# AshuiRUA/NPI-GNN

Hardware: AMD Instinct MI355X
Metric: edges/sec per GNN layer (fwd+bwd) (higher is better)
Workload: dtype f32; 1 GPU; C4 synthetic ncRNA-protein bipartite graph, N=1000000 nodes, E=20000000 directed edges (both directions, Zipf-skewed protein side), 1 SAGEConv layer 256->256 fp32, fwd+bwd incl. dX/dW/db, graph+features resident in HBM; parallelism=single GPU, hip_graph_replay=False, setup_steps=40, csr_sorted_columns=True

## Files before the change

include/npi_gnn.h:

```cpp
#ifndef NPI_GNN_H
#define NPI_GNN_H

#include <stdint.h>

#ifdef __cplusplus
extern "C" {
#endif

#define NPI_OK 0
#define NPI_ERR_ARG (-1)
#define NPI_ERR_LAUNCH (-2)
#define NPI_ERR_WORKSPACE (-3)

#ifndef NPI_ITEM_EDGES
#define NPI_ITEM_EDGES 256
#endif

#define NPI_F32 0
#define NPI_BF16 1

const char* npi_last_error(void);
int npi_abi_version(void);

int64_t npi_csr_workspace_bytes(int64_t E, int64_t N);
// ... 5 lines not shown
int npi_csr_build_ex(const int64_t* key_nodes, const int64_t* val_nodes, int64_t E, int64_t N,
                     int64_t n_cols, int add_self_loops, int64_t loop_col_offset, int build_flags,
                     int32_t* rowptr, int32_t* col, int32_t* eid, int32_t* rowidx,
                     int32_t* item_row, int64_t item_edges, int32_t* status,
                     void* workspace, int64_t workspace_bytes, void* stream);

int npi_edge_positions(const int32_t* eid, const int32_t* rowptr, int64_t N, int64_t nnz_max,
                       int64_t E, int32_t* pos_of, void* stream);

int64_t npi_segsum_carry_elems(int64_t nnz_max, int64_t item_edges, int64_t F);
int npi_segsum_scales_supported(int64_t F, int dtype);
int npi_segsum_ex(const int32_t* rowptr, const int32_t* col, const int32_t* item_row, int64_t item_edges,
                   const float* w, int64_t N, int64_t nnz_max, const void* x, int64_t ldx,
                   const void* x2, int64_t split, void* out, int64_t ldo, int64_t F, int dtype, int mean,
                   const float* bias, float* carry, float* row_scales_out, void* stream);

int npi_row_weight_sum(const int32_t* rowptr, const float* w, int64_t N, float* deg, void* stream);
int npi_gcn_norm(const int32_t* rowidx, const int32_t* col, const int32_t* rowptr, const float* w,
                 const float* deg, const int32_t* deg_rowptr, int64_t N, int64_t nnz_max, float* norm,
                 void* stream);
int npi_entry_col_scale(const int32_t* col, const int32_t* rowptr, const float* table, const float* w_in, int64_t N, int64_t n_cols,
                        int64_t nnz_max, float* w_out, void* stream);
int npi_row_inv_count(const int32_t* rowptr, int64_t N, float* inv_cnt, void* stream);
int npi_entry_weights(const int32_t* eid, const int32_t* rowidx, const int32_t* rowptr,
                      const float* edge_w, const float* loop_w_node, float fill,
                      int64_t N, int64_t nnz_max, float* w_entry, void* stream);
int npi_hold_cus(int workgroups, int64_t nanoseconds, uint64_t* start_word, void* stream);
int npi_relu_backward(const float* dy, int64_t ldd, const float* y, int64_t ldy, int64_t M, int64_t F, float* dz, int64_t ldz,
                      void* stream);

// ... 189 lines not shown
```

npi_gnn_amd/_lib.py:

```python
from __future__ import annotations

import ctypes
import os
from ctypes import c_char_p, c_float, c_int, c_int64, c_void_p

import torch

HERE = os.path.dirname(os.path.abspath(__file__))
LIB_PATH = os.environ.get("NPI_GNN_LIB") or os.path.join(HERE, "libnpi_gnn.so")

NPI_F32 = 0
NPI_BF16 = 1
NPI_GEMM_EXACT_F32 = 1
NPI_GEMM_SPLIT_BF16 = 2
NPI_GEMM_A_ZERO_PADDED = 4
NPI_GEMM_WORKSPACE_PREPARED = 8
NPI_GEMM_SPLIT_F16X2 = 16
NPI_PREPARE_F16X2 = 4


def NPI_GEMM_RESERVE_CUS(n: int) -> int:
    n = int(n)
    if n < 0 or n > 128 or n % 8:
        raise ValueError(f"NPI_GEMM_RESERVE_CUS: a multiple of 8 in [0, 128], got {n}")
    return (n // 8) << 8

_P = c_void_p
_I = c_int64

PROTOTYPES = {
    "npi_last_error": (c_char_p, []),
    "npi_abi_version": (c_int, []),
    "npi_csr_workspace_bytes": (_I, [_I, _I]),
    "npi_item_edges": (_I, [_I]),
    "npi_num_items": (_I, [_I, _I]),
    "npi_csr_build_ex": (c_int, [_P, _P, _I, _I, _I, c_int, _I, c_int, _P, _P, _P, _P, _P, _I, _P, _P, _I, _P]),
    "npi_edge_positions": (c_int, [_P, _P, _I, _I, _I, _P, _P]),
    "npi_segsum_carry_elems": (_I, [_I, _I, _I]),
    "npi_segsum_ex": (c_int, [_P, _P, _P, _I, _P, _I, _I, _P, _I, _P, _I, _P, _I, _I, c_int, c_int, _P, _P, _P, _P]),
    "npi_segsum_scales_supported": (c_int, [_I, c_int]),
    "npi_row_weight_sum": (c_int, [_P, _P, _I, _P, _P]),
    "npi_gcn_norm": (c_int, [_P, _P, _P, _P, _P, _P, _I, _I, _P, _P]),
    "npi_row_inv_count": (c_int, [_P, _I, _P, _P]),
    "npi_entry_col_scale": (c_int, [_P, _P, _P, _P, _I, _I, _I, _P, _P]),
    "npi_entry_weights": (c_int, [_P, _P, _P, _P, _P, c_float, _I, _I, _P, _P]),
    "npi_relu_backward": (c_int, [_P, _I, _P, _I, _I, _I, _P, _I, _P]),
    "npi_l2_normalize_rows": (c_int, [_P, _I, _I, _I, c_float, _P, _I, _P, _P]),
    "npi_l2_normalize_rows_bwd": (c_int, [_P, _I, _P, _I, _P, _I, _I, c_float, _P, _I, _P]),
    "npi_colsum_workspace_elems": (_I, [_I, _I]),
    "npi_colsum": (c_int, [_P, _I, _I, _I, _P, _P, _I, _P]),
    "npi_linear_bwd_weight_workspace_elems": (_I, [_I, _I, _I]),
    "npi_linear_workspace_bytes": (_I, [_I, _I]),
    "npi_row_scales": (c_int, [_P, _I, _I, _I, _P, _P]),
    "npi_linear_fwd_ex": (c_int, [_P, _I, _P, _I, _P, _P, _P, _I, _I, _I, _I, c_int, c_int, c_int, _P, _I, _P, _P]),
    "npi_linear_bwd_data_ex": (c_int, [_P, _I, _P, _I, _P, _P, _I, _I, _I, _I, c_int, c_int, _P, _I, _P, _P]),
# ... 124 lines not shown
```

npi_gnn_amd/build.py:

```python
from __future__ import annotations

import os
import shutil
import subprocess
import sys

HERE = os.path.dirname(os.path.abspath(__file__))
CSRC = os.path.join(HERE, "csrc")
LIB = os.path.join(HERE, "libnpi_gnn.so")
SOURCES = ["csr_build.hip", "segsum.hip", "gemm_f32.hip", "graph_ops.hip", "gat.hip", "segscan.hip", "pool.hip", "subgraph.hip",
           "head.hip", "layer.hip"]
HOST_ONLY = {"layer.hip"}
ARCH = "gfx950"


def _hipcc() -> str:
    for cand in (os.environ.get("HIPCC"), shutil.which("hipcc"), "/opt/rocm/bin/hipcc"):
        if cand and os.path.exists(cand):
            return cand
    raise RuntimeError("hipcc not found (expected /opt/rocm/bin/hipcc)")


MANIFEST = os.path.join(HERE, "build", "manifest.json")


# ... 64 lines not shown
```

npi_gnn_amd/csrc/csr_build.hip:

```cpp
#include "npi_common.h"
#include <stdarg.h>

namespace npi {

static thread_local char g_err[512] = "";
void set_error(const char* fmt, ...) {
    va_list ap;
    va_start(ap, fmt);
    vsnprintf(g_err, sizeof(g_err), fmt, ap);
    va_end(ap);
}

constexpr int SORT_THREADS = 256;
constexpr int SORT_WAVES = SORT_THREADS / WAVE;
constexpr int SORT_ITEMS = 16;
constexpr int SORT_WAVE_TILE = WAVE * SORT_ITEMS;
constexpr int SORT_TILE = SORT_THREADS * SORT_ITEMS;
constexpr int RADIX = 256;

constexpr int SCAN_THREADS = 256;
constexpr int SCAN_ITEMS = 8;
constexpr int SCAN_TILE = SCAN_THREADS * SCAN_ITEMS;
static_assert(SCAN_THREADS == SORT_THREADS && SORT_THREADS == 256, "one thread per radix digit");

// ... 579 lines not shown
    if (n_out == 0) {
        (void)hipMemsetAsync(rowptr_o, 0, sizeof(int32_t), stream);
    } else {
        const unsigned tiles = (unsigned)ceil_div(n_out, 256);
        int32_t* cnt = workspace;
        int32_t* tile_total = workspace + n_out;
        csr_filter_count_kernel<<<tiles, 256, 0, stream>>>(rowptr, col, perm, remap, (int)n_out, cnt, tile_total);
        csr_filter_fill_kernel<<<tiles, 256, 0, stream>>>(rowptr, col, eid, perm, remap, newpos, (int)n_out, cnt, tile_total,
                                                          rowptr_o, col_o, eid_o, rowidx_o);
    }
    const int64_t n_items = num_items_of(nnz_max_out, item_edges);
    item_rows_kernel<<<(unsigned)ceil_div(n_items + 1, 256), 256, 0, stream>>>(rowptr_o, n_out, n_items, (int)item_edges, item_row_o);
    return check_launch("npi_csr_filter");
}

extern "C" int npi_edge_positions(const int32_t* eid, const int32_t* rowptr, int64_t N, int64_t nnz_max,
                                  int64_t E, int32_t* pos_of, void* stream_) {
    hipStream_t stream = (hipStream_t)stream_;
    NPI_REQUIRE(E >= 0 && nnz_max >= 0, "npi_edge_positions: negative size");
    if (E > 0) fill_i32_kernel<<<(unsigned)ceil_div(E, 256), 256, 0, stream>>>(pos_of, E, -1);
    if (nnz_max > 0)
        edge_positions_kernel<<<(unsigned)ceil_div(nnz_max, 256), 256, 0, stream>>>(eid, rowptr, N, nnz_max, pos_of);
    return check_launch("npi_edge_positions");
}
```

npi_gnn_amd/functional.py:

```python
from __future__ import annotations

from typing import Optional

import torch

from ._lib import (NPI_BF16, NPI_F32, NPI_GEMM_A_ZERO_PADDED, NPI_GEMM_EXACT_F32, NPI_GEMM_RESERVE_CUS, NPI_GEMM_SPLIT_F16X2,
                   NPI_GEMM_WORKSPACE_PREPARED, NPI_PREPARE_F16X2, check, load, ptr, require_gpu, stream_ptr)
from .graph import CSRGraph, CSRSide, as_graph
from .schedule import DEFAULT, Schedule


_PROFILE = None
_PROFILE_TAGS = None


class _tag_events:

    def __init__(self, tag, dev):
        self.rec = _PROFILE_TAGS
        if self.rec is not None:
            self.tag, self.dev = tag, dev
            self.e0, self.e1 = torch.cuda.Event(enable_timing=True), torch.cuda.Event(enable_timing=True)

    def __enter__(self):
# ... 73 lines not shown
def _check_out(out: torch.Tensor, rows: int, cols: int, like: torch.Tensor, what: str) -> None:
    if (out.dim() != 2 or out.size(0) != rows or out.size(1) != cols or out.dtype != like.dtype or out.stride(1) != 1
            or out.device != like.device):
        raise ValueError(f"{what}: out must be [{rows}, {cols}] {like.dtype} with unit column stride on {like.device} "
                         f"(got {tuple(out.shape)} {out.dtype}, strides {tuple(out.stride())}, {out.device})")


def segsum_scales_ok(side: CSRSide, x: torch.Tensor, out: Optional[torch.Tensor] = None) -> bool:
    return (x.dtype == torch.float32 and x.size(1) == 256 and side.nnz_max > 0 and x.stride(0) % 4 == 0 and x.data_ptr() % 16 == 0
            and (out is None or (out.stride(0) % 4 == 0 and out.data_ptr() % 16 == 0)))


def segsum(graph: CSRGraph, side: CSRSide, x: torch.Tensor, w: Optional[torch.Tensor] = None,
           mean: bool = False, bias: Optional[torch.Tensor] = None,
           out: Optional[torch.Tensor] = None, x2: Optional[torch.Tensor] = None,
           scales_out: Optional[torch.Tensor] = None) -> torch.Tensor:
    dev = require_gpu(x, w, bias, x2)
    x = _fcp(x, "x")
    if bias is not None:
        bias = _fc(bias, "bias", x)
    N, F = side.n_rows, x.size(1)
    split = x.size(0)
    if x2 is not None:
        x2 = _fc(x2, "x2", x)
        if x2.size(1) != F:
            raise ValueError("x2 must have the width of x")
        if x2.stride(0) != x.stride(0):
            x2 = x2.contiguous()
            if x2.stride(0) != x.stride(0):
                x = x.contiguous()
    if side.n_cols > split + (x2.size(0) if x2 is not None else 0):
        raise ValueError(f"the table has {split + (x2.size(0) if x2 is not None else 0)} rows, the adjacency indexes {side.n_cols}")
    if out is None:
        out = torch.empty((N, F), dtype=x.dtype, device=dev)
    else:
        _check_out(out, N, F, x, "segsum")
    carry = side.carry(F)
    prof = _PROFILE
    if prof is not None:
        ev0, ev1 = torch.cuda.Event(enable_timing=True), torch.cuda.Event(enable_timing=True)
        ev0.record(torch.cuda.current_stream(dev))
    if scales_out is not None and (scales_out.dtype != torch.float32 or scales_out.numel() != N or not scales_out.is_contiguous()):
        raise ValueError("segsum: scales_out must be a contiguous float32 vector with one element per output row")
    check(load().npi_segsum_ex(ptr(side.rowptr), ptr(side.col), ptr(side.item_row), side.item, ptr(w), N, side.nnz_max,
                                ptr(x), x.stride(0), ptr(x2), split if x2 is not None else 0, ptr(out), out.stride(0), F,
                                _code(x), 1 if mean else 0, ptr(bias), ptr(carry), ptr(scales_out), stream_ptr(dev)), "npi_segsum")
    if prof is not None:
        ev1.record(torch.cuda.current_stream(dev))
        prof.append((ev0, ev1))
    return out




def _gflags(sch: Schedule) -> int:
    return NPI_GEMM_EXACT_F32 if sch.gemm_exact_f32 else 0


def _f16x2(sch: Schedule, rows: int, K: int, N: int, dtype) -> bool:
    return (sch.f16x2_min_rows is not None and not sch.gemm_exact_f32 and rows >= sch.f16x2_min_rows and dtype == torch.float32
            and f16x2_shape(rows, K, N))


def _gemm_workspace(K: int, N: int, dev) -> torch.Tensor:
    return torch.empty(int(load().npi_linear_workspace_bytes(K, N)), dtype=torch.uint8, device=dev)
# ... 428 lines not shown
    inv = graph.inv_count(graph.by_dst)
    out = torch.empty(max(tside.nnz_max, 1), dtype=torch.float32, device=dev)
    check(load().npi_entry_col_scale(ptr(tside.col), ptr(tside.rowptr), ptr(inv), ptr(w_src), tside.n_rows, inv.numel(), tside.nnz_max,
                                     ptr(out), stream_ptr(dev)), "npi_entry_col_scale")
    if w_src is None:
        cache[key] = out
    return out


def _aggregate_first_ok(sch: Schedule, f16: bool, weight: torch.Tensor, grad_out: torch.Tensor, tside: CSRSide, ws_bwd) -> bool:
    return (sch.aggregate_first_backward and f16 and isinstance(ws_bwd, Planes) and ws_bwd.f16 and grad_out.dtype == torch.float32 and grad_out.size(1) == 256
            and segsum_scales_ok(tside, grad_out) and f16x2_shape(grad_out.size(0), grad_out.size(1), weight.size(0)))


def _backward_aggregate_first(graph, tside: CSRSide, w_t: Optional[torch.Tensor], agg, weight, grad_out, ws_bwd: "Planes", want_w: bool,
                              has_bias: bool, overlap: bool, k_valid=None):
    dev = grad_out.device
    N, Nout = grad_out.shape
    t = torch.empty((N, Nout), dtype=torch.float32, device=dev)
    t_scales = torch.empty(N, dtype=torch.float32, device=dev)
    dw = db = None
    if overlap and want_w:
        main = torch.cuda.current_stream(dev)
        side = _side_stream(dev)
        side.wait_stream(main)
        dw, db = linear_bwd_weight(agg, grad_out, want_bias=has_bias, shared=True, k_valid=k_valid)
        with torch.cuda.stream(side):
            segsum(graph, tside, grad_out, w=w_t, mean=False, out=t, scales_out=t_scales)
        for buf in (grad_out, t, t_scales):
            buf.record_stream(side)
        main.wait_stream(side)
    else:
        if want_w:
            dw, db = linear_bwd_weight(agg, grad_out, want_bias=has_bias, k_valid=k_valid)
        segsum(graph, tside, grad_out, w=w_t, mean=False, out=t, scales_out=t_scales)
    dx = linear_bwd_data(t, weight, ws=ws_bwd, dc_scales=t_scales)
    return dx, dw, db


class _SageConvFn(torch.autograd.Function):
    @staticmethod
    def forward(ctx, x, weight, bias, graph: CSRGraph, w_entry=None, relu: bool = False, sch: Schedule = DEFAULT):
        ctx.graph = graph
        ctx.w_src = w_entry[1] if w_entry else None
        ctx.has_bias = bias is not None
        ctx.relu = relu
        ctx.sch = sch
        ctx.k_rows = None
        f16 = (x.dtype == weight.dtype and x.size(1) == weight.size(0)
               and _f16x2(sch, graph.by_dst.n_rows, weight.size(0), weight.size(1), x.dtype) and segsum_scales_ok(graph.by_dst, x))
        ctx.f16 = f16
        if f16:
            agg = torch.empty((graph.by_dst.n_rows, x.size(1)), dtype=x.dtype, device=x.device)
            scales = torch.empty(agg.size(0), dtype=torch.float32, device=x.device)
            segsum(graph, graph.by_dst, x, w=w_entry[0] if w_entry else None, mean=True, out=agg, scales_out=scales)
            wsf, ctx.ws_bwd = prepare_weight(weight, backward=ctx.needs_input_grad[0], f16=True)
            out = linear_fwd(agg, weight, bias, relu=relu, ws=wsf, a_scales=scales)
            ctx.k_valid = None
            ctx.save_for_backward(agg, weight, *([out] if relu else []))
            return out
        fl = _gflags(sch)
        if not fl and _layer_calls_ok() and x.dtype == weight.dtype and x.dtype in (torch.float32, torch.bfloat16) and not (
                x.dtype == torch.bfloat16 and weight.size(0) % 128 != 0 and 2 * _pad128(weight.size(0)) <= 3 * weight.size(0)):
            agg, out, ctx.ws_bwd = conv_fwd(graph.by_dst, x, w_entry[0] if w_entry else None, True, weight, bias, relu,
                                            ctx.needs_input_grad[0])
            ctx.k_valid = weight.size(0) if agg.size(1) != weight.size(0) else None
            ctx.save_for_backward(agg, weight, *([out] if relu else []))
            return out
        agg = None if fl else padded_aggregate_buffer(x, weight.size(0), graph.by_dst.n_rows, bf16_ok=True)
        if agg is None:
            agg = segsum(graph, graph.by_dst, x, w=w_entry[0] if w_entry else None, mean=True)
        else:
            segsum(graph, graph.by_dst, x, w=w_entry[0] if w_entry else None, mean=True, out=agg[:, : x.size(1)])
        if agg.size(1) != weight.size(0) and agg.dtype == torch.bfloat16:
            ctx.k_rows = weight.size(0)
            weight = torch.nn.functional.pad(weight.detach(), (0, 0, 0, agg.size(1) - weight.size(0)))
        wsf, ctx.ws_bwd = prepare_weight(weight, backward=ctx.needs_input_grad[0]) if (
            agg.size(1) == weight.size(0) and agg.dtype == weight.dtype and not fl) else (None, None)
        out = linear_fwd(agg, weight, bias, relu=relu, ws=wsf, flags=fl)
        ctx.k_valid = weight.size(0) if agg.size(1) != weight.size(0) else None
        ctx.save_for_backward(agg, weight, *([out] if relu else []))
        return out

    @staticmethod
    def backward(ctx, grad_out):
        agg, weight = ctx.saved_tensors[:2]
# ... 7 lines not shown
        if not fl and not overlap and ctx.k_rows is None and _layer_calls_ok() and (want_w or want_x) and not ctx.f16:
            out_relu = None
            if ctx.relu:
                if grad_out.dtype == torch.float32:
                    out_relu = ctx.saved_tensors[2]
                else:
                    grad_out = relu_backward(grad_out, ctx.saved_tensors[2])
            dx, dw, db = conv_bwd(tside() if want_x else graph.by_dst, grad_out, out_relu, agg, weight, graph.inv_count(graph.by_dst),
                                  ctx.w_src, ctx.ws_bwd, want_x, want_w, ctx.has_bias)
            return dx, dw, db, None, None, None, None
        if ctx.relu:
            grad_out = relu_backward(grad_out, ctx.saved_tensors[2])
        dx = dw = db = None
        if want_x and _aggregate_first_ok(ctx.sch, ctx.f16, weight, grad_out, tside(), ctx.ws_bwd):
            ts = tside()
            dx, dw, db = _backward_aggregate_first(graph, ts, mean_bwd_weights(graph, ts, ctx.w_src), agg, weight, grad_out, ctx.ws_bwd,
                                                   want_w, ctx.has_bias, overlap, ctx.k_valid)
            return dx, dw, db, None, None, None, None
        ws_bwd = ctx.ws_bwd if not (isinstance(ctx.ws_bwd, Planes) and ctx.ws_bwd.f16) else None
        if want_w and not overlap:
            dw, db = linear_bwd_weight(agg, grad_out, want_bias=ctx.has_bias, k_valid=ctx.k_valid, flags=fl)
        if want_x:
            dagg = linear_bwd_data(grad_out, weight, rowscale=graph.inv_count(graph.by_dst), ws=ws_bwd, flags=fl)
            if ctx.k_rows is not None:
                dagg = dagg[:, : ctx.k_rows]
            if overlap:
                dev = grad_out.device
                main = torch.cuda.current_stream(dev)
                side = _side_stream(dev)
                side.wait_stream(main)
                dw, db = linear_bwd_weight(agg, grad_out, want_bias=ctx.has_bias, shared=True, k_valid=ctx.k_valid, flags=fl)
                with torch.cuda.stream(side):
                    dx = segsum(graph, tside(), dagg, w=ctx.w_src, mean=False)
                dagg.record_stream(side)
                dx.record_stream(main)
                main.wait_stream(side)
            else:
                dx = segsum(graph, tside(), dagg, w=ctx.w_src, mean=False)
        if dw is not None and ctx.k_rows is not None:
            dw = dw[: ctx.k_rows]
        return dx, dw, db, None, None, None, None


class _SageConcatFn(torch.autograd.Function):

    @staticmethod
    def forward(ctx, x, weight, bias, graph: CSRGraph, w_entry=None):
        N, F = x.shape
        cat = torch.empty((N, 2 * F), dtype=x.dtype, device=x.device)
        cat[:, :F].copy_(x)
        segsum(graph, graph.by_dst, x, w=w_entry[0] if w_entry else None, mean=True, out=cat[:, F:])
        out = linear_fwd(cat, weight, bias)
        ctx.graph, ctx.F = graph, F
# ... 724 lines not shown
```

npi_gnn_amd/graph.py:

```python
from __future__ import annotations

from dataclasses import dataclass, field
from typing import Dict, Optional

import torch

from . import _lib
from ._lib import check, load, ptr, require_gpu, stream_ptr

_DEBUG = False

_PENDING = []
_PENDING_MAX = 256


def set_debug(flag: bool) -> None:
    global _DEBUG
    _DEBUG = bool(flag)


def pending_status(device=None) -> list:
    if device is None:
        out = list(_PENDING)
        _PENDING.clear()
# ... 40 lines not shown
@dataclass
class CSRSide:
    rowptr: torch.Tensor
    col: torch.Tensor
    eid: torch.Tensor
    rowidx: torch.Tensor
    item_row: torch.Tensor
    status: torch.Tensor
    nnz_max: int
    n_items: int
    _inv_cnt: Optional[torch.Tensor] = None
    _carry: Dict[tuple, torch.Tensor] = field(default_factory=dict)
    n_rows: int = -1
    n_cols: int = -1
    item: int = 0

    def inv_count(self) -> torch.Tensor:
        if self._inv_cnt is None:
            dev = self.rowptr.device
            out = torch.empty(self.n_rows, dtype=torch.float32, device=dev)
            check(load().npi_row_inv_count(ptr(self.rowptr), self.n_rows, ptr(out), stream_ptr(dev)),
                  "npi_row_inv_count")
            self._inv_cnt = out
        return self._inv_cnt

    def carry(self, F: int) -> torch.Tensor:
        dev = self.rowptr.device
        key = (F, _lib.stream_ptr(dev))
        buf = self._carry.pop(key, None)
        if buf is None:
            n = int(load().npi_segsum_carry_elems(self.nnz_max, self.item, F))
            buf = torch.zeros(n, dtype=torch.float32, device=dev)
            if len(self._carry) >= CARRY_SLOTS and not torch.cuda.is_current_stream_capturing():
                self._carry.pop(next(iter(self._carry)))
        elif _DEBUG and not torch.cuda.is_current_stream_capturing():
            self._check_counters(buf)
        self._carry[key] = buf
        return buf

    def _check_counters(self, buf: torch.Tensor) -> None:
        n_wg = -(-self.n_items // 4)
        n = n_wg + 2 * (-(-n_wg // 64))
        if n and int(buf[:n].view(torch.int32).abs().max()) != 0:
            raise _lib.NpiError("aggregation scratch: an arrival counter is not zero between launches -- two launches shared the "
                                "buffer concurrently or one was aborted; call reset_carry() on this side")

    def reset_carry(self) -> None:
        self._carry.clear()


def item_hint(nnz_max: int) -> int:
    return int(load().npi_item_edges(int(nnz_max)))


def build_side(key: torch.Tensor, val: torch.Tensor, n_rows: int, n_cols: int, self_loops: bool = True,
               loop_col_offset: int = 0, drop_equal: bool = True, item: Optional[int] = None,
               sort_columns: bool = False) -> CSRSide:
    lib = load()
    dev = require_gpu(key, val)
    E, N = int(key.numel()), int(n_rows)
    nnz_max = E + (N if self_loops else 0)
    item = item_hint(nnz_max) if item is None else int(item)
    n_items = int(lib.npi_num_items(nnz_max, item))
# ... 9 lines not shown
    ws_bytes = int(lib.npi_csr_workspace_bytes(E, N))
    ws = torch.empty(ws_bytes, dtype=torch.uint8, device=dev)
    check(lib.npi_csr_build_ex(ptr(key), ptr(val), E, N, int(n_cols), 1 if self_loops else 0,
                               int(loop_col_offset), (1 if drop_equal else 0) | (2 if sort_columns else 0), ptr(rowptr), ptr(col), ptr(eid),
                               ptr(rowidx), ptr(item_row), item, ptr(status), ptr(ws), ws_bytes, stream_ptr(dev)),
          "npi_csr_build_ex")
    note_status(status)
    side = CSRSide(rowptr, col, eid, rowidx, item_row, status, nnz_max, n_items)
    side.n_rows, side.n_cols, side.item = N, int(n_cols), item
    return side


class CSRGraph:

    def __init__(self, edge_index: torch.Tensor, num_nodes: int, self_loops: bool = True, by_dst: Optional[CSRSide] = None,
                 symmetric: bool = False, item: Optional[int] = None, sort_columns: bool = False, keep_equal: bool = False):
        if edge_index.dtype != torch.int64 or edge_index.dim() != 2 or edge_index.size(0) != 2:
            raise ValueError("edge_index must be a LongTensor of shape [2, E]")
        require_gpu(edge_index)
        self.num_nodes = int(num_nodes)
        self.num_edges = int(edge_index.size(1))
        self.self_loops = bool(self_loops)
        self.device = edge_index.device
        self._ei_version = edge_index._version
        self._ei_ptr = edge_index.data_ptr()
        self.symmetric = bool(symmetric)
        self._src = edge_index[0].contiguous()
        self._dst = edge_index[1].contiguous()
        self._item = item if by_dst is None else by_dst.item
        self.sort_columns = bool(sort_columns)
        self.keep_equal = bool(keep_equal)
        if self.keep_equal and self.self_loops:
            raise ValueError("CSRGraph: keep_equal=True (existing self loops stay ordinary entries) needs self_loops=False")
        self.by_dst = by_dst if by_dst is not None else \
            build_side(self._dst, self._src, self.num_nodes, self.num_nodes, self.self_loops, drop_equal=not self.keep_equal,
                       item=self._item, sort_columns=self.sort_columns)
        self._by_src: Optional[CSRSide] = None

    @property
    def by_src(self) -> CSRSide:
        if self._by_src is None:
            self._by_src = build_side(self._src, self._dst, self.num_nodes, self.num_nodes, self.self_loops,
                                      drop_equal=not self.keep_equal, item=self.by_dst.item, sort_columns=self.sort_columns)
        return self._by_src

    def built_from(self, edge_index: torch.Tensor, num_nodes: Optional[int] = None) -> bool:
# ... 159 lines not shown
```

Before: 3.207 billion edges/s.

## Stream hub rows as dense masked column scan instead of CSR gather

Picks up to 128 highest-degree rows (hubs) of the CSR side and builds a per-column bitmask of which hubs touch each column. A new streaming kernel walks the feature table once in slabs and accumulates all hub rows at the same time from shared-memory tiles. The remaining light rows are aggregated by the existing segsum on a reduced CSR. This targets the cost of Zipf-skewed hub rows, which cause long serial gathers and load imbalance. In exchange it adds a full dense pass over X, partial buffers and a finalize step, plus a one-time planning cost and a host sync when the plan is built.

```diff
diff --git a/include/npi_gnn.h b/include/npi_gnn.h
--- a/include/npi_gnn.h
+++ b/include/npi_gnn.h
@@ -43,6 +43,20 @@
                    const float* w, int64_t N, int64_t nnz_max, const void* x, int64_t ldx,
                    const void* x2, int64_t split, void* out, int64_t ldo, int64_t F, int dtype, int mean,
                    const float* bias, float* carry, float* row_scales_out, void* stream);
+
+#define NPI_HUB_MAX 128
+int64_t npi_hub_plan_workspace_elems(void);
+int npi_hub_plan(const int32_t* rowptr, const int32_t* col, int64_t N, int64_t n_cols, int64_t nnz_max, int64_t h_max,
+                 int64_t min_degree, int64_t min_entries, int32_t* hub_rows, uint32_t* mask, int32_t* info, int32_t* workspace,
+                 void* stream);
+int npi_hub_light_side(const int32_t* rowptr, const int32_t* col, const int32_t* eid, const int32_t* rowidx, int64_t N,
+                       int64_t nnz_max, const int32_t* hub_rows, int64_t H, int64_t nnz_max_light, int64_t item_edges,
+                       int32_t* rowptr_l, int32_t* col_l, int32_t* eid_l, int32_t* rowidx_l, int32_t* item_row_l, void* stream);
+int64_t npi_segsum_hub_slabs(int64_t n_cols);
+int64_t npi_segsum_hub_partial_elems(int64_t n_cols);
+int npi_segsum_hub(const int32_t* hub_rows, int64_t H, const uint32_t* mask, const int32_t* rowptr, int64_t N, int64_t n_cols,
+                   const float* col_scale, const float* x, int64_t ldx, float* out, int64_t ldo, int64_t F, int mean,
+                   float* partial, float* row_scales_out, void* stream);
 
 int npi_row_weight_sum(const int32_t* rowptr, const float* w, int64_t N, float* deg, void* stream);
 int npi_gcn_norm(const int32_t* rowidx, const int32_t* col, const int32_t* rowptr, const float* w,
diff --git a/npi_gnn_amd/_lib.py b/npi_gnn_amd/_lib.py
--- a/npi_gnn_amd/_lib.py
+++ b/npi_gnn_amd/_lib.py
@@ -17,6 +17,7 @@
 NPI_GEMM_WORKSPACE_PREPARED = 8
 NPI_GEMM_SPLIT_F16X2 = 16
 NPI_PREPARE_F16X2 = 4
+NPI_HUB_MAX = 128
 
 
 def NPI_GEMM_RESERVE_CUS(n: int) -> int:
@@ -39,6 +40,12 @@
     "npi_segsum_carry_elems": (_I, [_I, _I, _I]),
     "npi_segsum_ex": (c_int, [_P, _P, _P, _I, _P, _I, _I, _P, _I, _P, _I, _P, _I, _I, c_int, c_int, _P, _P, _P, _P]),
     "npi_segsum_scales_supported": (c_int, [_I, c_int]),
+    "npi_hub_plan_workspace_elems": (_I, []),
+    "npi_hub_plan": (c_int, [_P, _P, _I, _I, _I, _I, _I, _I, _P, _P, _P, _P, _P]),
+    "npi_hub_light_side": (c_int, [_P, _P, _P, _P, _I, _I, _P, _I, _I, _I, _P, _P, _P, _P, _P, _P]),
+    "npi_segsum_hub_slabs": (_I, [_I]),
+    "npi_segsum_hub_partial_elems": (_I, [_I]),
+    "npi_segsum_hub": (c_int, [_P, _I, _P, _P, _I, _I, _P, _P, _I, _P, _I, _I, c_int, _P, _P, _P]),
     "npi_row_weight_sum": (c_int, [_P, _P, _I, _P, _P]),
     "npi_gcn_norm": (c_int, [_P, _P, _P, _P, _P, _P, _I, _I, _P, _P]),
     "npi_row_inv_count": (c_int, [_P, _I, _P, _P]),
diff --git a/npi_gnn_amd/build.py b/npi_gnn_amd/build.py
--- a/npi_gnn_amd/build.py
+++ b/npi_gnn_amd/build.py
@@ -8,7 +8,7 @@
 HERE = os.path.dirname(os.path.abspath(__file__))
 CSRC = os.path.join(HERE, "csrc")
 LIB = os.path.join(HERE, "libnpi_gnn.so")
-SOURCES = ["csr_build.hip", "segsum.hip", "gemm_f32.hip", "graph_ops.hip", "gat.hip", "segscan.hip", "pool.hip", "subgraph.hip",
+SOURCES = ["csr_build.hip", "segsum.hip", "segsum_hub.hip", "gemm_f32.hip", "graph_ops.hip", "gat.hip", "segscan.hip", "pool.hip", "subgraph.hip",
            "head.hip", "layer.hip"]
 HOST_ONLY = {"layer.hip"}
 ARCH = "gfx950"
diff --git a/npi_gnn_amd/csrc/csr_build.hip b/npi_gnn_amd/csrc/csr_build.hip
--- a/npi_gnn_amd/csrc/csr_build.hip
+++ b/npi_gnn_amd/csrc/csr_build.hip
@@ -617,6 +617,177 @@
     return check_launch("npi_csr_filter");
 }
 
+namespace npi {
+
+constexpr int HUB_CAND_CAP = 4096;
+constexpr int HUB_WS_CNT = 0, HUB_WS_IDENT = 1, HUB_WS_PRELIM = 8, HUB_WS_BAD = HUB_WS_PRELIM + NPI_HUB_MAX,
+              HUB_WS_REMAP = HUB_WS_BAD + NPI_HUB_MAX, HUB_WS_CAND = HUB_WS_REMAP + NPI_HUB_MAX, HUB_WS_ELEMS = HUB_WS_CAND + HUB_CAND_CAP;
+constexpr int HUB_WORDS = NPI_HUB_MAX / 32;
+
+__global__ void hub_candidates_kernel(const int32_t* __restrict__ rowptr, int64_t N, int32_t min_degree, int32_t* __restrict__ ws) {
+    int64_t r = (int64_t)blockIdx.x * blockDim.x + threadIdx.x;
+    if (r >= N || rowptr[r + 1] - rowptr[r] < min_degree) return;
+    const int i = atomicAdd(&ws[HUB_WS_CNT], 1);
+    if (i < HUB_CAND_CAP) ws[HUB_WS_CAND + i] = (int32_t)r;
+}
+
+__global__ void __launch_bounds__(1024)
+hub_select_kernel(const int32_t* __restrict__ rowptr, int h_max, int32_t* __restrict__ ws, int32_t* __restrict__ info) {
+    __shared__ int32_t rows[HUB_CAND_CAP], degs[HUB_CAND_CAP];
+    const int seen = ws[HUB_WS_CNT];
+    const int n = seen > HUB_CAND_CAP ? 0 : seen;
+    for (int c = threadIdx.x; c < n; c += blockDim.x) {
+        const int32_t r = ws[HUB_WS_CAND + c];
+        rows[c] = r;
+        degs[c] = rowptr[r + 1] - rowptr[r];
+    }
+    __syncthreads();
+    for (int c = threadIdx.x; c < n; c += blockDim.x) {
+        const int32_t r = rows[c], d = degs[c];
+        int rank = 0;
+        for (int o = 0; o < n; ++o) rank += (degs[o] > d || (degs[o] == d && rows[o] < r)) ? 1 : 0;
+        if (rank < h_max) ws[HUB_WS_PRELIM + rank] = r;
+    }
+    if (threadIdx.x == 0) {
+        info[2] = seen;
+        info[3] = n < h_max ? n : h_max;
+    }
+    if (threadIdx.x < NPI_HUB_MAX) ws[HUB_WS_BAD + threadIdx.x] = 0;
+}
+
+__global__ void __launch_bounds__(256)
+hub_mask_kernel(const int32_t* __restrict__ rowptr, const int32_t* __restrict__ col, int64_t n_cols, int32_t* __restrict__ ws,
+                const int32_t* __restrict__ info, uint32_t* __restrict__ mask) {
+    const int j = blockIdx.y;
+    if (j >= info[3]) return;
+    const int32_t r = ws[HUB_WS_PRELIM + j];
+    const uint32_t bit = 1u << (j & 31);
+    const int64_t p1 = rowptr[r + 1];
+    for (int64_t p = (int64_t)rowptr[r] + blockIdx.x * 256 + threadIdx.x; p < p1; p += (int64_t)gridDim.x * 256) {
+        const int32_t c = col[p];
+        if (c < 0 || c >= n_cols) { ws[HUB_WS_BAD + j] = 1; continue; }
+        const uint32_t old = atomicOr(&mask[(int64_t)c * HUB_WORDS + (j >> 5)], bit);
+        if (old & bit) ws[HUB_WS_BAD + j] = 1;
+    }
+}
+
+__global__ void hub_finalize_kernel(const int32_t* __restrict__ rowptr, int64_t min_entries, int32_t* __restrict__ ws,
+                                    int32_t* __restrict__ info, int32_t* __restrict__ hub_rows) {
+    if (threadIdx.x != 0 || blockIdx.x != 0) return;
+    const int h0 = info[3];
+    int h = 0;
+    int64_t total = 0;
+    for (int j = 0; j < NPI_HUB_MAX; ++j) {
+        int m = -1;
+        if (j < h0 && ws[HUB_WS_BAD + j] == 0) {
+            const int32_t r = ws[HUB_WS_PRELIM + j];
+            hub_rows[h] = r;
+            total += rowptr[r + 1] - rowptr[r];
+            m = h++;
+        }
+        ws[HUB_WS_REMAP + j] = m;
+    }
+    if (total < min_entries || total >= ((int64_t)1 << 31)) h = 0;
+    for (int j = h; j < NPI_HUB_MAX; ++j) hub_rows[j] = -1;
+    ws[HUB_WS_IDENT] = (h == h0) ? 1 : 0;
+    info[0] = h;
+    info[1] = h > 0 ? (int32_t)total : 0;
+}
+
+__global__ void hub_mask_remap_kernel(int64_t n_cols, const int32_t* __restrict__ ws, const int32_t* __restrict__ info,
+                                      uint32_t* __restrict__ mask) {
+    if (ws[HUB_WS_IDENT] != 0 || info[0] == 0) return;
+    int64_t c = (int64_t)blockIdx.x * blockDim.x + threadIdx.x;
+    if (c >= n_cols) return;
+    uint32_t out[HUB_WORDS] = {};
+    bool any = false;
+    for (int q = 0; q < HUB_WORDS; ++q) {
+        uint32_t m = mask[c * HUB_WORDS + q];
+        any |= m != 0u;
+        while (m != 0u) {
+            const int b = __builtin_ctz(m);
+            m &= m - 1u;
+            const int nj = ws[HUB_WS_REMAP + q * 32 + b];
+            if (nj >= 0) out[nj >> 5] |= 1u << (nj & 31);
+        }
+    }
+    if (!any) return;
+    for (int q = 0; q < HUB_WORDS; ++q) mask[c * HUB_WORDS + q] = out[q];
+}
+
+__global__ void __launch_bounds__(256)
+hub_light_rowptr_kernel(const int32_t* __restrict__ rowptr, int64_t N, const int32_t* __restrict__ hub_rows, int H,
+                        int32_t* __restrict__ rowptr_l) {
+    __shared__ int32_t hr[NPI_HUB_MAX], hd[NPI_HUB_MAX];
+    if (threadIdx.x < H) {
+        const int32_t r = hub_rows[threadIdx.x];
+        hr[threadIdx.x] = r;
+        hd[threadIdx.x] = rowptr[r + 1] - rowptr[r];
+    }
+    __syncthreads();
+    int64_t r = (int64_t)blockIdx.x * 256 + threadIdx.x;
+    if (r > N) return;
+    int32_t removed = 0;
+    for (int j = 0; j < H; ++j) removed += (hr[j] < r) ? hd[j] : 0;
+    rowptr_l[r] = rowptr[r] - removed;
+}
+
+__global__ void hub_light_entries_kernel(const int32_t* __restrict__ rowptr, const int32_t* __restrict__ col,
+                                         const int32_t* __restrict__ eid, const int32_t* __restrict__ rowidx, int64_t N, int64_t nnz_max,
+                                         const int32_t* __restrict__ rowptr_l, int64_t nnz_max_l, int32_t* __restrict__ col_l,
+                                         int32_t* __restrict__ eid_l, int32_t* __restrict__ rowidx_l) {
+    int64_t p = (int64_t)blockIdx.x * blockDim.x + threadIdx.x;
+    if (p >= nnz_max || p >= rowptr[N]) return;
+    const int32_t r = rowidx[p];
+    if (r < 0 || r >= N || rowptr_l[r + 1] == rowptr_l[r]) return;
+    const int64_t q = p - (rowptr[r] - rowptr_l[r]);
+    if (q < 0 || q >= nnz_max_l) return;
+    col_l[q] = col[p];
+    eid_l[q] = eid[p];
+    rowidx_l[q] = r;
+}
+
+}
+
+extern "C" int64_t npi_hub_plan_workspace_elems(void) { return HUB_WS_ELEMS; }
+
+extern "C" int npi_hub_plan(const int32_t* rowptr, const int32_t* col, int64_t N, int64_t n_cols, int64_t nnz_max, int64_t h_max,
+                            int64_t min_degree, int64_t min_entries, int32_t* hub_rows, uint32_t* mask, int32_t* info,
+                            int32_t* workspace, void* stream_) {
+    hipStream_t stream = (hipStream_t)stream_;
+    NPI_REQUIRE(N > 0 && n_cols > 0 && nnz_max > 0 && N < ((int64_t)1 << 31) && n_cols < ((int64_t)1 << 31), "npi_hub_plan: bad size");
+    NPI_REQUIRE(h_max >= 1 && h_max <= NPI_HUB_MAX, "npi_hub_plan: h_max must be in [1, NPI_HUB_MAX]");
+    NPI_REQUIRE(min_degree >= 1 && min_degree < ((int64_t)1 << 31) && min_entries >= 0, "npi_hub_plan: bad threshold");
+    NPI_REQUIRE(rowptr && col && hub_rows && mask && info && workspace, "npi_hub_plan: null pointer");
+    (void)hipMemsetAsync(workspace, 0, HUB_WS_CAND * sizeof(int32_t), stream);
+    (void)hipMemsetAsync(info, 0, 4 * sizeof(int32_t), stream);
+    (void)hipMemsetAsync(mask, 0, (size_t)n_cols * HUB_WORDS * sizeof(uint32_t), stream);
+    hub_candidates_kernel<<<(unsigned)ceil_div(N, 256), 256, 0, stream>>>(rowptr, N, (int32_t)min_degree, workspace);
+    hub_select_kernel<<<1, 1024, 0, stream>>>(rowptr, (int)h_max, workspace, info);
+    hub_mask_kernel<<<dim3(64, NPI_HUB_MAX), 256, 0, stream>>>(rowptr, col, n_cols, workspace, info, mask);
+    hub_finalize_kernel<<<1, 64, 0, stream>>>(rowptr, min_entries, workspace, info, hub_rows);
+    hub_mask_remap_kernel<<<(unsigned)ceil_div(n_cols, 256), 256, 0, stream>>>(n_cols, workspace, info, mask);
+    return check_launch("npi_hub_plan");
+}
+
+extern "C" int npi_hub_light_side(const int32_t* rowptr, const int32_t* col, const int32_t* eid, const int32_t* rowidx, int64_t N,
+                                  int64_t nnz_max, const int32_t* hub_rows, int64_t H, int64_t nnz_max_light, int64_t item_edges,
+                                  int32_t* rowptr_l, int32_t* col_l, int32_t* eid_l, int32_t* rowidx_l, int32_t* item_row_l,
+                                  void* stream_) {
+    hipStream_t stream = (hipStream_t)stream_;
+    NPI_REQUIRE(N > 0 && nnz_max > 0 && nnz_max_light >= 0 && nnz_max_light <= nnz_max, "npi_hub_light_side: bad size");
+    NPI_REQUIRE(H >= 1 && H <= NPI_HUB_MAX, "npi_hub_light_side: H must be in [1, NPI_HUB_MAX]");
+    NPI_REQUIRE(item_edges_ok(item_edges), "npi_hub_light_side: item_edges must be 64 or NPI_ITEM_EDGES");
+    NPI_REQUIRE(rowptr && col && eid && rowidx && hub_rows && rowptr_l && col_l && eid_l && rowidx_l && item_row_l,
+                "npi_hub_light_side: null pointer");
+    hub_light_rowptr_kernel<<<(unsigned)ceil_div(N + 1, 256), 256, 0, stream>>>(rowptr, N, hub_rows, (int)H, rowptr_l);
+    hub_light_entries_kernel<<<(unsigned)ceil_div(nnz_max, 256), 256, 0, stream>>>(rowptr, col, eid, rowidx, N, nnz_max, rowptr_l,
+                                                                                 nnz_max_light, col_l, eid_l, rowidx_l);
+    const int64_t n_items = num_items_of(nnz_max_light, item_edges);
+    item_rows_kernel<<<(unsigned)ceil_div(n_items + 1, 256), 256, 0, stream>>>(rowptr_l, N, n_items, (int)item_edges, item_row_l);
+    return check_launch("npi_hub_light_side");
+}
+
 extern "C" int npi_edge_positions(const int32_t* eid, const int32_t* rowptr, int64_t N, int64_t nnz_max,
                                   int64_t E, int32_t* pos_of, void* stream_) {
     hipStream_t stream = (hipStream_t)stream_;
diff --git a/npi_gnn_amd/csrc/segsum_hub.hip b/npi_gnn_amd/csrc/segsum_hub.hip
--- /dev/null
+++ b/npi_gnn_amd/csrc/segsum_hub.hip
@@ -0,0 +1,169 @@
+#include "npi_common.h"
+
+namespace npi {
+
+constexpr int HUB_WAVES = 8;
+constexpr int HUB_PER_WAVE = NPI_HUB_MAX / HUB_WAVES;
+constexpr int HUB_THREADS = HUB_WAVES * WAVE;
+constexpr int HUB_TILE = 32;
+constexpr int HUB_TILE_LOADS = HUB_TILE / HUB_WAVES;
+constexpr int HUB_SLAB = 2048;
+constexpr int HUB_F = 256;
+constexpr int HUB_MASK_WORDS = NPI_HUB_MAX / 32;
+constexpr int FIN_WAVES = 16;
+static_assert(HUB_PER_WAVE == 16 && HUB_MASK_WORDS == 4, "the wave's 16 mask bits are cut out of four 32-bit words");
+static_assert(HUB_TILE == 32 && HUB_TILE % HUB_WAVES == 0, "one mask row per lane of a half wave");
+
+__device__ __forceinline__ uint32_t wave_pattern(const uint4& m, int w) {
+    return ((m.x >> w) & 0x01010101u) | (((m.y >> w) & 0x01010101u) << 1) | (((m.z >> w) & 0x01010101u) << 2) |
+           (((m.w >> w) & 0x01010101u) << 3);
+}
+constexpr uint32_t pattern_bit(int k) { return 1u << (8 * (k & 3) + (k >> 2)); }
+__device__ __forceinline__ int hub_of(int k, int w) { return ((k >> 2) * 32) + (k & 3) * 8 + w; }
+
+__device__ __forceinline__ void hub_prefetch(const float* __restrict__ x, int64_t ldx, const uint4* __restrict__ mask,
+                                             const float* __restrict__ col_scale, int t0, int r1, int w, int lane,
+                                             float4 (&pre)[HUB_TILE_LOADS], uint32_t& pat_n, uint32_t& need_n, float& cs_n) {
+    const int row = t0 + lane;
+    const bool valid = lane < HUB_TILE && row < r1;
+    uint4 m = make_uint4(0u, 0u, 0u, 0u);
+    if (valid) m = mask[row];
+    cs_n = (valid && col_scale != nullptr) ? col_scale[row] : 1.f;
+    pat_n = wave_pattern(m, w);
+    need_n = (uint32_t)__ballot((m.x | m.y | m.z | m.w) != 0u);
+#pragma unroll
+    for (int t = 0; t < HUB_TILE_LOADS; ++t) {
+        const int i = w + HUB_WAVES * t;
+        if ((need_n >> i) & 1u)
+            pre[t] = *reinterpret_cast<const float4*>(x + (int64_t)(t0 + i) * ldx + lane * 4);
+    }
+}
+
+__global__ void __launch_bounds__(HUB_THREADS, 4)
+hub_stream_kernel(const float* __restrict__ x, int64_t ldx, const uint4* __restrict__ mask, const float* __restrict__ col_scale,
+                  int n_cols, int H, float* __restrict__ partial) {
+    __shared__ float4 tile[HUB_TILE][WAVE];
+    const int lane = lane_id();
+    const int w = uniform_i(threadIdx.x >> 6);
+    const int r0 = blockIdx.x * HUB_SLAB;
+    const int r1 = min(r0 + HUB_SLAB, n_cols);
+
+    float4 acc[HUB_PER_WAVE];
+#pragma unroll
+    for (int k = 0; k < HUB_PER_WAVE; ++k) acc[k] = make_float4(0.f, 0.f, 0.f, 0.f);
+
+    float4 pre[HUB_TILE_LOADS];
+#pragma unroll
+    for (int t = 0; t < HUB_TILE_LOADS; ++t) pre[t] = make_float4(0.f, 0.f, 0.f, 0.f);
+    uint32_t pat_n = 0, need_n = 0;
+    float cs_n = 1.f;
+    if (r0 < r1) hub_prefetch(x, ldx, mask, col_scale, r0, r1, w, lane, pre, pat_n, need_n, cs_n);
+    for (int t0 = r0; t0 < r1; t0 += HUB_TILE) {
+        __syncthreads();
+#pragma unroll
+        for (int t = 0; t < HUB_TILE_LOADS; ++t) {
+            const int i = w + HUB_WAVES * t;
+            if ((need_n >> i) & 1u) tile[i][lane] = pre[t];
+        }
+        const uint32_t pat = pat_n;
+        const float cs = cs_n;
+        __syncthreads();
+        if (t0 + HUB_TILE < r1) hub_prefetch(x, ldx, mask, col_scale, t0 + HUB_TILE, r1, w, lane, pre, pat_n, need_n, cs_n);
+#pragma unroll
+        for (int k = 0; k < HUB_PER_WAVE; ++k) {
+            uint32_t m = (uint32_t)__ballot((pat & pattern_bit(k)) != 0u);
+            while (m != 0u) {
+                const int i = uniform_i(__builtin_ctz(m));
+                m &= m - 1u;
+                const float s = bcast_f(cs, i);
+                const float4 v = tile[i][lane];
+                acc[k].x = fmaf(v.x, s, acc[k].x);
+                acc[k].y = fmaf(v.y, s, acc[k].y);
+                acc[k].z = fmaf(v.z, s, acc[k].z);
+                acc[k].w = fmaf(v.w, s, acc[k].w);
+            }
+        }
+    }
+    float4* __restrict__ dst = reinterpret_cast<float4*>(partial) + (int64_t)blockIdx.x * NPI_HUB_MAX * WAVE;
+#pragma unroll
+    for (int k = 0; k < HUB_PER_WAVE; ++k) {
+        const int j = hub_of(k, w);
+        if (j < H) dst[(int64_t)j * WAVE + lane] = acc[k];
+    }
+}
+
+__device__ __forceinline__ float4 add4(const float4& a, const float4& b) { return make_float4(a.x + b.x, a.y + b.y, a.z + b.z, a.w + b.w); }
+
+__global__ void __launch_bounds__(FIN_WAVES * WAVE)
+hub_finish_kernel(const float* __restrict__ partial, int n_slabs, const int32_t* __restrict__ hub_rows, const int32_t* __restrict__ rowptr,
+                  int mean, float* __restrict__ out, int64_t ldo, float* __restrict__ scale_out) {
+    __shared__ float4 part[FIN_WAVES][WAVE];
+    const int lane = lane_id();
+    const int w = uniform_i(threadIdx.x >> 6);
+    const int j = blockIdx.x;
+    const int chunk = (n_slabs + FIN_WAVES - 1) / FIN_WAVES;
+    const int s0 = w * chunk, s1 = min(s0 + chunk, n_slabs);
+    const float4* __restrict__ src = reinterpret_cast<const float4*>(partial) + (int64_t)j * WAVE + lane;
+    const int64_t step = (int64_t)NPI_HUB_MAX * WAVE;
+    float4 a = make_float4(0.f, 0.f, 0.f, 0.f);
+    int s = s0;
+    for (; s + 8 <= s1; s += 8) {
+        float4 v[8];
+#pragma unroll
+        for (int u = 0; u < 8; ++u) v[u] = src[(int64_t)(s + u) * step];
+#pragma unroll
+        for (int u = 0; u < 8; ++u) a = add4(a, v[u]);
+    }
+    for (; s < s1; ++s) a = add4(a, src[(int64_t)s * step]);
+    part[w][lane] = a;
+    __syncthreads();
+    if (w != 0) return;
+    a = part[0][lane];
+#pragma unroll
+    for (int g = 1; g < FIN_WAVES; ++g) a = add4(a, part[g][lane]);
+    const int r = hub_rows[j];
+    float sc = 1.f;
+    if (mean) sc = 1.f / (float)max(rowptr[r + 1] - rowptr[r], 1);
+    const float4 t = make_float4(fmaf(a.x, sc, 0.f), fmaf(a.y, sc, 0.f), fmaf(a.z, sc, 0.f), fmaf(a.w, sc, 0.f));
+    *reinterpret_cast<float4*>(out + (int64_t)r * ldo + lane * 4) = t;
+    if (scale_out != nullptr) {
+        float m = fmaxf(fmaxf(fabsf(t.x), fabsf(t.y)), fmaxf(fabsf(t.z), fabsf(t.w)));
+#pragma unroll
+        for (int o = 32; o >= 1; o >>= 1) m = fmaxf(m, __shfl_xor(m, o));
+        if (lane == 0) scale_out[r] = pow2_scale_of(m);
+    }
+}
+
+}
+
+using namespace npi;
+
+extern "C" int64_t npi_segsum_hub_slabs(int64_t n_cols) { return n_cols <= 0 ? 0 : ceil_div(n_cols, HUB_SLAB); }
+
+extern "C" int64_t npi_segsum_hub_partial_elems(int64_t n_cols) {
+    return n_cols < 0 ? -1 : (npi_segsum_hub_slabs(n_cols) > 0 ? npi_segsum_hub_slabs(n_cols) : 1) * NPI_HUB_MAX * HUB_F;
+}
+
+extern "C" int npi_segsum_hub(const int32_t* hub_rows, int64_t H, const uint32_t* mask, const int32_t* rowptr, int64_t N, int64_t n_cols,
+                              const float* col_scale, const float* x, int64_t ldx, float* out, int64_t ldo, int64_t F, int mean,
+                              float* partial, float* row_scales_out, void* stream_) {
+    hipStream_t stream = (hipStream_t)stream_;
+    NPI_REQUIRE(H >= 0 && H <= NPI_HUB_MAX, "npi_segsum_hub: H must be in [0, NPI_HUB_MAX]");
+    NPI_REQUIRE(F == HUB_F, "npi_segsum_hub: f32 rows of 256 columns only");
+    NPI_REQUIRE(N >= 0 && n_cols >= 0 && n_cols < ((int64_t)1 << 31) - HUB_SLAB, "npi_segsum_hub: bad size");
+    if (H == 0) return NPI_OK;
+    NPI_REQUIRE(hub_rows && mask && rowptr && x && out && partial, "npi_segsum_hub: null pointer");
+    NPI_REQUIRE(ldx >= F && ldo >= F && ldx % 4 == 0 && ldo % 4 == 0 && ((uintptr_t)x % 16) == 0 && ((uintptr_t)out % 16) == 0 &&
+                    ((uintptr_t)partial % 16) == 0 && ((uintptr_t)mask % 16) == 0,
+                "npi_segsum_hub: rows and masks must be 16-byte aligned");
+    const int64_t n_slabs = npi_segsum_hub_slabs(n_cols);
+    if (n_slabs > 0) {
+        hipLaunchKernelGGL(hub_stream_kernel, dim3((unsigned)n_slabs), dim3(HUB_THREADS), 0, stream, x, ldx,
+                           reinterpret_cast<const uint4*>(mask), col_scale, (int)n_cols, (int)H, partial);
+        int rc = check_launch("npi_segsum_hub(stream)");
+        if (rc != NPI_OK) return rc;
+    }
+    hipLaunchKernelGGL(hub_finish_kernel, dim3((unsigned)H), dim3(FIN_WAVES * WAVE), 0, stream, partial, (int)n_slabs, hub_rows, rowptr,
+                       mean, out, ldo, row_scales_out);
+    return check_launch("npi_segsum_hub(finish)");
+}
diff --git a/npi_gnn_amd/functional.py b/npi_gnn_amd/functional.py
--- a/npi_gnn_amd/functional.py
+++ b/npi_gnn_amd/functional.py
@@ -6,7 +6,7 @@
 
 from ._lib import (NPI_BF16, NPI_F32, NPI_GEMM_A_ZERO_PADDED, NPI_GEMM_EXACT_F32, NPI_GEMM_RESERVE_CUS, NPI_GEMM_SPLIT_F16X2,
                    NPI_GEMM_WORKSPACE_PREPARED, NPI_PREPARE_F16X2, check, load, ptr, require_gpu, stream_ptr)
-from .graph import CSRGraph, CSRSide, as_graph
+from .graph import CSRGraph, CSRSide, HubPlan, as_graph
 from .schedule import DEFAULT, Schedule
 
 
@@ -111,8 +111,9 @@
 def segsum(graph: CSRGraph, side: CSRSide, x: torch.Tensor, w: Optional[torch.Tensor] = None,
            mean: bool = False, bias: Optional[torch.Tensor] = None,
            out: Optional[torch.Tensor] = None, x2: Optional[torch.Tensor] = None,
-           scales_out: Optional[torch.Tensor] = None) -> torch.Tensor:
-    dev = require_gpu(x, w, bias, x2)
+           scales_out: Optional[torch.Tensor] = None, hub: Optional[HubPlan] = None,
+           col_scale: Optional[torch.Tensor] = None) -> torch.Tensor:
+    dev = require_gpu(x, w, bias, x2, col_scale)
     x = _fcp(x, "x")
     if bias is not None:
         bias = _fc(bias, "bias", x)
@@ -132,6 +133,18 @@
         out = torch.empty((N, F), dtype=x.dtype, device=dev)
     else:
         _check_out(out, N, F, x, "segsum")
+    full = side
+    if hub is not None:
+        if not (x.dtype == torch.float32 and F == 256 and x2 is None and bias is None and x.stride(0) % 4 == 0 and x.data_ptr() % 16 == 0
+                and out.stride(0) % 4 == 0 and out.data_ptr() % 16 == 0 and hub.light.n_rows == N):
+            raise ValueError("segsum(hub=): the streaming path takes one f32 table of 256 columns, 16-byte aligned rows, no bias")
+        if col_scale is not None:
+            col_scale = _f32c(col_scale, "col_scale")
+            if col_scale.numel() != side.n_cols:
+                raise ValueError(f"segsum: col_scale has {col_scale.numel()} elements, the table {side.n_cols} rows")
+        side = hub.light
+    elif col_scale is not None:
+        raise ValueError("segsum: col_scale belongs to the streaming path (hub=); the plain launch takes per-entry weights")
     carry = side.carry(F)
     prof = _PROFILE
     if prof is not None:
@@ -142,10 +155,20 @@
     check(load().npi_segsum_ex(ptr(side.rowptr), ptr(side.col), ptr(side.item_row), side.item, ptr(w), N, side.nnz_max,
                                 ptr(x), x.stride(0), ptr(x2), split if x2 is not None else 0, ptr(out), out.stride(0), F,
                                 _code(x), 1 if mean else 0, ptr(bias), ptr(carry), ptr(scales_out), stream_ptr(dev)), "npi_segsum")
+    if hub is not None:
+        check(load().npi_segsum_hub(ptr(hub.hub_rows), hub.H, ptr(hub.mask), ptr(full.rowptr), N, full.n_cols, ptr(col_scale), ptr(x),
+                                    x.stride(0), ptr(out), out.stride(0), F, 1 if mean else 0, ptr(hub.partial()), ptr(scales_out),
+                                    stream_ptr(dev)), "npi_segsum_hub")
     if prof is not None:
         ev1.record(torch.cuda.current_stream(dev))
         prof.append((ev0, ev1))
     return out
+
+
+def hub_plan_for(graph: CSRGraph, side: CSRSide, x: torch.Tensor, out: Optional[torch.Tensor] = None) -> Optional[HubPlan]:
+    if not graph.hub_stream or not segsum_scales_ok(side, x, out) or x.size(0) != side.n_cols:
+        return None
+    return side.hub_plan()
 
 
 
@@ -604,8 +627,9 @@
 
 
 def _backward_aggregate_first(graph, tside: CSRSide, w_t: Optional[torch.Tensor], agg, weight, grad_out, ws_bwd: "Planes", want_w: bool,
-                              has_bias: bool, overlap: bool, k_valid=None):
+                              has_bias: bool, overlap: bool, k_valid=None, hub: Optional[HubPlan] = None):
     dev = grad_out.device
+    cs = graph.inv_count(graph.by_dst) if hub is not None else None
     N, Nout = grad_out.shape
     t = torch.empty((N, Nout), dtype=torch.float32, device=dev)
     t_scales = torch.empty(N, dtype=torch.float32, device=dev)
@@ -616,14 +640,14 @@
         side.wait_stream(main)
         dw, db = linear_bwd_weight(agg, grad_out, want_bias=has_bias, shared=True, k_valid=k_valid)
         with torch.cuda.stream(side):
-            segsum(graph, tside, grad_out, w=w_t, mean=False, out=t, scales_out=t_scales)
+            segsum(graph, tside, grad_out, w=w_t, mean=False, out=t, scales_out=t_scales, hub=hub, col_scale=cs)
         for buf in (grad_out, t, t_scales):
             buf.record_stream(side)
         main.wait_stream(side)
     else:
         if want_w:
             dw, db = linear_bwd_weight(agg, grad_out, want_bias=has_bias, k_valid=k_valid)
-        segsum(graph, tside, grad_out, w=w_t, mean=False, out=t, scales_out=t_scales)
+        segsum(graph, tside, grad_out, w=w_t, mean=False, out=t, scales_out=t_scales, hub=hub, col_scale=cs)
     dx = linear_bwd_data(t, weight, ws=ws_bwd, dc_scales=t_scales)
     return dx, dw, db
 
@@ -643,7 +667,8 @@
         if f16:
             agg = torch.empty((graph.by_dst.n_rows, x.size(1)), dtype=x.dtype, device=x.device)
             scales = torch.empty(agg.size(0), dtype=torch.float32, device=x.device)
-            segsum(graph, graph.by_dst, x, w=w_entry[0] if w_entry else None, mean=True, out=agg, scales_out=scales)
+            hub = hub_plan_for(graph, graph.by_dst, x, agg) if not w_entry else None
+            segsum(graph, graph.by_dst, x, w=w_entry[0] if w_entry else None, mean=True, out=agg, scales_out=scales, hub=hub)
             wsf, ctx.ws_bwd = prepare_weight(weight, backward=ctx.needs_input_grad[0], f16=True)
             out = linear_fwd(agg, weight, bias, relu=relu, ws=wsf, a_scales=scales)
             ctx.k_valid = None
@@ -659,7 +684,8 @@
             return out
         agg = None if fl else padded_aggregate_buffer(x, weight.size(0), graph.by_dst.n_rows, bf16_ok=True)
         if agg is None:
-            agg = segsum(graph, graph.by_dst, x, w=w_entry[0] if w_entry else None, mean=True)
+            agg = segsum(graph, graph.by_dst, x, w=w_entry[0] if w_entry else None, mean=True,
+                         hub=hub_plan_for(graph, graph.by_dst, x) if not w_entry else None)
         else:
             segsum(graph, graph.by_dst, x, w=w_entry[0] if w_entry else None, mean=True, out=agg[:, : x.size(1)])
         if agg.size(1) != weight.size(0) and agg.dtype == torch.bfloat16:
@@ -697,8 +723,10 @@
         dx = dw = db = None
         if want_x and _aggregate_first_ok(ctx.sch, ctx.f16, weight, grad_out, tside(), ctx.ws_bwd):
             ts = tside()
-            dx, dw, db = _backward_aggregate_first(graph, ts, mean_bwd_weights(graph, ts, ctx.w_src), agg, weight, grad_out, ctx.ws_bwd,
-                                                   want_w, ctx.has_bias, overlap, ctx.k_valid)
+            hub = hub_plan_for(graph, ts, grad_out) if ctx.w_src is None else None
+            w_t = mean_bwd_weights(graph, ts if hub is None else hub.light, ctx.w_src)
+            dx, dw, db = _backward_aggregate_first(graph, ts, w_t, agg, weight, grad_out, ctx.ws_bwd, want_w, ctx.has_bias, overlap,
+                                                   ctx.k_valid, hub=hub)
             return dx, dw, db, None, None, None, None
         ws_bwd = ctx.ws_bwd if not (isinstance(ctx.ws_bwd, Planes) and ctx.ws_bwd.f16) else None
         if want_w and not overlap:
@@ -714,12 +742,14 @@
                 side.wait_stream(main)
                 dw, db = linear_bwd_weight(agg, grad_out, want_bias=ctx.has_bias, shared=True, k_valid=ctx.k_valid, flags=fl)
                 with torch.cuda.stream(side):
-                    dx = segsum(graph, tside(), dagg, w=ctx.w_src, mean=False)
+                    dx = segsum(graph, tside(), dagg, w=ctx.w_src, mean=False,
+                                hub=hub_plan_for(graph, tside(), dagg) if ctx.w_src is None else None)
                 dagg.record_stream(side)
                 dx.record_stream(main)
                 main.wait_stream(side)
             else:
-                dx = segsum(graph, tside(), dagg, w=ctx.w_src, mean=False)
+                dx = segsum(graph, tside(), dagg, w=ctx.w_src, mean=False,
+                            hub=hub_plan_for(graph, tside(), dagg) if ctx.w_src is None else None)
         if dw is not None and ctx.k_rows is not None:
             dw = dw[: ctx.k_rows]
         return dx, dw, db, None, None, None, None
diff --git a/npi_gnn_amd/graph.py b/npi_gnn_amd/graph.py
--- a/npi_gnn_amd/graph.py
+++ b/npi_gnn_amd/graph.py
@@ -78,6 +78,8 @@
     n_rows: int = -1
     n_cols: int = -1
     item: int = 0
+    _hub: Optional["HubPlan"] = None
+    _hub_asked: bool = False
 
     def inv_count(self) -> torch.Tensor:
         if self._inv_cnt is None:
@@ -87,6 +89,15 @@
                   "npi_row_inv_count")
             self._inv_cnt = out
         return self._inv_cnt
+
+    def hub_plan(self) -> Optional["HubPlan"]:
+        if not self._hub_asked:
+            if self.n_rows != self.n_cols or self.n_cols < HUB_MIN_COLS or self.nnz_max <= 0:
+                self._hub_asked = True
+            elif not torch.cuda.is_current_stream_capturing():
+                self._hub = build_hub_plan(self)
+                self._hub_asked = True
+        return self._hub
 
     def carry(self, F: int) -> torch.Tensor:
         dev = self.rowptr.device
@@ -111,6 +122,72 @@
 
     def reset_carry(self) -> None:
         self._carry.clear()
+
+
+HUB_MIN_COLS = 262_144
+HUB_DEGREE_DIV = 512
+HUB_ENTRIES_PER_STREAMED_ROW = 2
+
+
+@dataclass
+class HubPlan:
+    H: int
+    n_entries: int
+    hub_rows: torch.Tensor
+    mask: torch.Tensor
+    light: CSRSide
+    _partial: Dict[int, torch.Tensor] = field(default_factory=dict)
+
+    def partial(self) -> torch.Tensor:
+        dev = self.mask.device
+        key = _lib.stream_ptr(dev)
+        buf = self._partial.pop(key, None)
+        if buf is None:
+            buf = torch.empty(int(load().npi_segsum_hub_partial_elems(self.mask.size(0))), dtype=torch.float32, device=dev)
+            if len(self._partial) >= CARRY_SLOTS and not torch.cuda.is_current_stream_capturing():
+                self._partial.pop(next(iter(self._partial)))
+        self._partial[key] = buf
+        return buf
+
+
+def build_hub_plan(side: CSRSide, h_max: int = _lib.NPI_HUB_MAX, min_degree: Optional[int] = None,
+                   min_entries: Optional[int] = None) -> Optional[HubPlan]:
+    if side.n_rows != side.n_cols:
+        raise ValueError("build_hub_plan: one-table sides with n_cols == n_rows only")
+    lib = load()
+    dev = side.rowptr.device
+    N = side.n_rows
+    if N <= 0 or side.nnz_max <= 0:
+        return None
+    if min_degree is None:
+        min_degree = max(-(-side.n_cols // HUB_DEGREE_DIV), 2)
+    if min_entries is None:
+        min_entries = HUB_ENTRIES_PER_STREAMED_ROW * side.n_cols
+    i32 = dict(dtype=torch.int32, device=dev)
+    hub_rows = torch.empty(_lib.NPI_HUB_MAX, **i32)
+    mask = torch.empty((side.n_cols, _lib.NPI_HUB_MAX // 32), **i32)
+    info = torch.empty(4, **i32)
+    ws = torch.empty(int(lib.npi_hub_plan_workspace_elems()), **i32)
+    s = stream_ptr(dev)
+    check(lib.npi_hub_plan(ptr(side.rowptr), ptr(side.col), N, side.n_cols, side.nnz_max, int(h_max), int(min_degree), int(min_entries),
+                           ptr(hub_rows), ptr(mask), ptr(info), ptr(ws), s), "npi_hub_plan")
+    H, n_entries = info.tolist()[:2]
+    if H == 0:
+        return None
+    nnz_max = side.nnz_max - n_entries
+    n_items = int(lib.npi_num_items(nnz_max, side.item))
+    rowptr = torch.empty(N + 1, **i32)
+    col = torch.empty(max(nnz_max, 1), **i32)
+    eid = torch.empty(max(nnz_max, 1), **i32)
+    rowidx = torch.empty(max(nnz_max, 1), **i32)
+    item_row = torch.empty(n_items + 1, **i32)
+    check(lib.npi_hub_light_side(ptr(side.rowptr), ptr(side.col), ptr(side.eid), ptr(side.rowidx), N, side.nnz_max, ptr(hub_rows), H,
+                                 nnz_max, side.item, ptr(rowptr), ptr(col), ptr(eid), ptr(rowidx), ptr(item_row), s),
+          "npi_hub_light_side")
+    light = CSRSide(rowptr, col, eid, rowidx, item_row, side.status, nnz_max, n_items)
+    light.n_rows, light.n_cols, light.item = N, side.n_cols, side.item
+    light._hub_asked = True
+    return HubPlan(H, n_entries, hub_rows, mask, light)
 
 
 def item_hint(nnz_max: int) -> int:
@@ -150,7 +227,8 @@
 class CSRGraph:
 
     def __init__(self, edge_index: torch.Tensor, num_nodes: int, self_loops: bool = True, by_dst: Optional[CSRSide] = None,
-                 symmetric: bool = False, item: Optional[int] = None, sort_columns: bool = False, keep_equal: bool = False):
+                 symmetric: bool = False, item: Optional[int] = None, sort_columns: bool = False, keep_equal: bool = False,
+                 hub_stream: bool = True):
         if edge_index.dtype != torch.int64 or edge_index.dim() != 2 or edge_index.size(0) != 2:
             raise ValueError("edge_index must be a LongTensor of shape [2, E]")
         require_gpu(edge_index)
@@ -166,6 +244,7 @@
         self._item = item if by_dst is None else by_dst.item
         self.sort_columns = bool(sort_columns)
         self.keep_equal = bool(keep_equal)
+        self.hub_stream = bool(hub_stream)
         if self.keep_equal and self.self_loops:
             raise ValueError("CSRGraph: keep_equal=True (existing self loops stay ordinary entries) needs self_loops=False")
         self.by_dst = by_dst if by_dst is not None else \
```

Result: faster. 3.598 billion edges/s (median of 6 runs) (+12.2%).
